# reinterpretcat/qwen3-rs

Hardware: NVIDIA B200
Metric: decode_tokens_per_s (higher is better)
Workload: dtype int8 weights x int8 activations, int32 group dots, f32 accumulate

## Files before the change

qwen3_rs_b200/csrc/q3_engine.cu:

```cuda
#include "../../include/qwen3_cuda.h"
#include "q3_kernels.cuh"
#include "q3_mega.cuh"
#include "q3_prefill.cuh"
#include "q3_sampler.cuh"
#include <cudaTypedefs.h>

#include <cuda_runtime.h>
#include <fcntl.h>
#include <math.h>
#include <stdarg.h>
#include <stdio.h>
#include <stdlib.h>
#include <string.h>
#include <sys/mman.h>
#include <sys/stat.h>
#include <unistd.h>

#include <string>
#include <vector>

using namespace q3;

static thread_local char g_err[1024] = "";
static int fail(int code, const char *fmt, ...) {
// ... 438 lines not shown
    }
    return 0;
}

template <class K>
static int allow_smem(K kernel, int bytes) {
    CK(cudaFuncSetAttribute(kernel, cudaFuncAttributeMaxDynamicSharedMemorySize, bytes));
    return 0;
}
static int prepare_exact_kernels() {
    int rc;
    if ((rc = allow_smem(k_rmsnorm_quant<32, true>, 65536))) return rc;
    if ((rc = allow_smem(k_rmsnorm_quant<64, true>, 65536))) return rc;
    if ((rc = allow_smem(k_rmsnorm_quant<128, true>, 65536))) return rc;
#define ALLOW_GEMV(GS)                                                      \
    if ((rc = allow_smem(k_gemv<GS, EPI_STORE, true, false>, 131072))) return rc;  \
    if ((rc = allow_smem(k_gemv<GS, EPI_QKV, true, false>, 131072))) return rc;    \
    if ((rc = allow_smem(k_gemv<GS, EPI_RESID, true, false>, 131072))) return rc;  \
    if ((rc = allow_smem(k_gemv<GS, EPI_SWIGLU, true, false>, 131072))) return rc; \
    if ((rc = allow_smem(k_gemv<GS, EPI_SWIGLU, true, true>, 131072))) return rc;  \
    if ((rc = allow_smem(k_gemv<GS, EPI_STORE, false, false>, 98304))) return rc;  \
    if ((rc = allow_smem(k_gemv<GS, EPI_QKV, false, false>, 98304))) return rc;    \
    if ((rc = allow_smem(k_gemv<GS, EPI_RESID, false, false>, 98304))) return rc;  \
    if ((rc = allow_smem(k_gemv<GS, EPI_SWIGLU, false, false>, 98304))) return rc; \
    if ((rc = allow_smem(k_gemv<GS, EPI_SWIGLU, false, true>, 98304))) return rc;
    ALLOW_GEMV(32)
    ALLOW_GEMV(64)
    ALLOW_GEMV(128)
#undef ALLOW_GEMV
    return 0;
}

static int pick_n_kt(int K, int gs) {
    for (int n = (K + MEGA_MAX_KT - 1) / MEGA_MAX_KT; n <= 64; n++)
        if (K % (n * gs) == 0 && (K / n) % 16 == 0 && K / n <= MEGA_MAX_KT) return n;
    return 0;
}

static int build_stream(q3_handle *h, MegaGemv &g, const std::vector<const DevQT *> &src, int units, int K, bool pair) {
    const int gs = h->cfg.group_size;
    g.units = units;
    g.K = K;
    g.n_kt = pick_n_kt(K, gs);
    if (!g.n_kt) return fail(Q3_EUNSUPPORTED, "no K tiling for K=%d gs=%d", K, gs);
    g.KT = K / g.n_kt;
    g.G = g.KT / gs;
    g.tile_bytes = g.KT + ((4 * g.G + 15) & ~15);
    const size_t rows = (size_t)units * (pair ? 2 : 1);
    g.layer_stride = (long long)(rows * g.n_kt * g.tile_bytes);
    uint8_t *buf = nullptr;
    int rc;
    if ((rc = dmalloc(h, (void **)&buf, (size_t)g.layer_stride * src.size()))) return rc;
    g.base = buf;
    for (size_t l = 0; l < src.size(); l++) {
        dim3 grid(units, g.n_kt);
        GS_DISPATCH(gs, (k_build_stream<GS><<<grid, 256, 0, h->stream>>>(src[l]->q, src[l]->s, buf + l * g.layer_stride, units, K,
                                                                        g.n_kt, h->num_sms, pair ? 1 : 0)));
    }
    CK(cudaGetLastError());
    return 0;
}

static PFN_cuTensorMapEncodeTiled_v12000 get_encode_fn();
static int make_map_kv(CUtensorMap *map, const float *base, size_t rows, int KV_l) {
    auto enc = get_encode_fn();
    if (!enc) return fail(Q3_ECUDA, "cuTensorMapEncodeTiled unavailable");
    cuuint64_t dims[2] = {(cuuint64_t)KV_l, (cuuint64_t)rows};
    cuuint64_t strides[1] = {(cuuint64_t)KV_l * 4};
    cuuint32_t box[2] = {(cuuint32_t)HEAD_DIM, (cuuint32_t)MEGA_KV_ROWS};
    cuuint32_t estr[2] = {1, 1};
    CUresult r = enc(map, CU_TENSOR_MAP_DATA_TYPE_FLOAT32, 2, const_cast<float *>(base), dims, strides, box, estr, CU_TENSOR_MAP_INTERLEAVE_NONE,
                     CU_TENSOR_MAP_SWIZZLE_NONE, CU_TENSOR_MAP_L2_PROMOTION_L2_128B, CU_TENSOR_MAP_FLOAT_OOB_FILL_NONE);
    if (r != CUDA_SUCCESS) return fail(Q3_ECUDA, "cuTensorMapEncodeTiled (KV cache) failed (%d) rows %zu KV %d", (int)r, rows, KV_l);
    return 0;
}

static int build_mega(q3_handle *h, const float *rms_att_all, const float *rms_ffn_all, const float *q_ln_all, const float *k_ln_all) {
    const q3_config &c = h->cfg;
    const int gs = c.group_size, L = c.n_layers, dim = c.dim;
    h->mega_ok = false;
    if (dim > MEGA_MAX_KT) { h->mega_why = "dim > 4096 (QKV/gate-up/lm_head phases need a single K tile)"; return 0; }
    if (!pick_n_kt(h->AH_l, gs) || !pick_n_kt(h->H_l, gs)) { h->mega_why = "no K tiling for o_proj/down"; return 0; }
    if (h->AH_l > 16384 || h->H_l > 16384 || dim > 16384) { h->mega_why = "activation vector > 16384"; return 0; }
    if (c.vocab_size % h->tp_size) { h->mega_why = "vocab not divisible by tp"; return 0; }
    if (h->layers[0].qkv.rows < h->num_sms || h->H_l < h->num_sms) { h->mega_why = "fewer qkv rows / FFN units than SMs"; return 0; }
    if (!get_encode_fn()) { h->mega_why = "cuTensorMapEncodeTiled unavailable"; return 0; }
    MegaArgs &a = h->margs;
    a = MegaArgs{};
    {
        int rck;
        if ((rck = make_map_kv(&a.map_k, h->kc, (size_t)L * c.seq_len, h->KV_l))) return rck;
        if ((rck = make_map_kv(&a.map_v, h->vc, (size_t)L * c.seq_len, h->KV_l))) return rck;
    }
    a.dim = dim; a.n_layers = L; a.n_heads_l = h->n_heads_l; a.n_kv_l = h->n_kv_l; a.AH_l = h->AH_l; a.KV_l = h->KV_l;
    a.H_l = h->H_l; a.seq_len = c.seq_len; a.tp_rank = h->tp_rank; a.tp_size = h->tp_size;
    a.vocab_l = c.vocab_size / h->tp_size;
    a.vocab_row0 = a.vocab_l * h->tp_rank;
    int rc;
    std::vector<const DevQT *> v;
    for (auto &W : h->layers) v.push_back(&W.qkv);
    if ((rc = build_stream(h, a.g[PH_QKV], v, h->layers[0].qkv.rows, dim, false))) return rc;
    v.clear();
    for (auto &W : h->layers) v.push_back(&W.wo);
    if ((rc = build_stream(h, a.g[PH_O], v, dim, h->AH_l, false))) return rc;
    v.clear();
    for (auto &W : h->layers) v.push_back(&W.w13);
    if ((rc = build_stream(h, a.g[PH_GU], v, h->H_l, dim, true))) return rc;
    v.clear();
    for (auto &W : h->layers) v.push_back(&W.w2);
    if ((rc = build_stream(h, a.g[PH_DN], v, dim, h->H_l, false))) return rc;
    DevQT head_slice = h->wcls;
    head_slice.q = h->wcls.q + (size_t)a.vocab_row0 * dim;
    head_slice.s = h->wcls.s + (size_t)a.vocab_row0 * (dim / gs);
    v.assign(1, &head_slice);
    if ((rc = build_stream(h, a.g[PH_HEAD], v, a.vocab_l, dim, false))) return rc;
    CK(cudaStreamSynchronize(h->stream));
    float *p;
    if ((rc = upload_f32(h, &p, rms_att_all, (size_t)L * dim))) return rc; a.rms_att = p;
    if ((rc = upload_f32(h, &p, rms_ffn_all, (size_t)L * dim))) return rc; a.rms_ffn = p;
    if ((rc = upload_f32(h, &p, q_ln_all, (size_t)L * HEAD_DIM))) return rc; a.q_ln = p;
    if ((rc = upload_f32(h, &p, k_ln_all, (size_t)L * HEAD_DIM))) return rc; a.k_ln = p;
    a.rms_final = h->rms_final;
    a.embed_q = h->embed.q; a.embed_s = h->embed.s; a.rope = h->rope; a.kc = h->kc; a.vc = h->vc;
    for (int i = 0; i < 2; i++) h->part_buf[i] = (unsigned long long *)(h->xchg + h->off_part[i]);
    {
        struct { unsigned long long **p; size_t words; } zones[] = {
            {&h->zq, (size_t)h->AH_l + 2 * (size_t)h->KV_l},
            {&h->za, (size_t)h->AH_l / 4 + (size_t)h->AH_l / gs},
            {&h->zh, (size_t)h->H_l},
            {&h->zr[0], (size_t)dim},
            {&h->zr[1], (size_t)dim}};
        for (auto &z : zones) {
            if ((rc = dmalloc(h, (void **)z.p, (z.words + 2) * 8))) return rc;
            CK(cudaMemset(*z.p, 0, (z.words + 2) * 8));
        }
    }
    h->d_best = (unsigned long long *)(h->xchg + h->off_best);
    h->d_flags = (unsigned int *)(h->xchg + h->off_flags);
    if ((rc = dmalloc(h, (void **)&h->d_bar, 64))) return rc;
    CK(cudaMemset(h->d_bar, 0, 64));
    if ((rc = dmalloc(h, (void **)&h->d_status, 64))) return rc;
    CK(cudaMemset(h->d_status, 0, 64));
    int *d_status = h->d_status;
    a.x = h->x;
    a.zq = h->zq; a.za = h->za; a.zh = h->zh; a.zr[0] = h->zr[0]; a.zr[1] = h->zr[1];
    a.attn_part = h->attn_part; a.att_cnt = h->att_cnt;
    a.bar = h->d_bar; a.status = d_status; a.tokpos = h->d_tokpos; a.history = h->d_history;
    for (int r = 0; r < MEGA_MAX_TP; r++) {
        a.part[0][r] = h->part_buf[0]; a.part[1][r] = h->part_buf[1];
        a.logits[r] = h->logits; a.best[r] = h->d_best; a.xbar[r] = (unsigned long long *)h->d_flags;
    }
    GS_DISPATCH(gs, KV_DISPATCH(h->kv_mul, (h->mega_fn = (void *)k_mega_decode<GS, KVM>)));
    if (!h->mega_fn) { h->mega_why = "no kernel for this GQA factor"; return 0; }
    const size_t slot = (size_t)MEGA_GW * (MEGA_MAX_KT + 4 * (MEGA_MAX_KT / gs));
    h->mega_smem = MEGA_NSTAGE * slot + MEGA_SCRATCH + 1024 + MEGA_MAX_KT * 4;
    CK(cudaFuncSetAttribute(h->mega_fn, cudaFuncAttributeMaxDynamicSharedMemorySize, (int)h->mega_smem));
    int occ = 0;
    CK(cudaOccupancyMaxActiveBlocksPerMultiprocessor(&occ, h->mega_fn, MEGA_THREADS, h->mega_smem));
    if (occ < 1) { h->mega_why = "megakernel does not fit on an SM"; return 0; }
    h->mega_ok = true;
    return 0;
}

static int launch_mega(q3_handle *h, int l0, int l1, bool from_embed, bool run_head, bool feedback, bool gather) {
    MegaArgs a = h->margs;
    a.layer0 = l0; a.layer1 = l1; a.from_embed = from_embed; a.run_head = run_head; a.feedback = feedback;
// ... 1399 lines not shown
```

qwen3_rs_b200/csrc/q3_mega.cuh:

```cuda
#pragma once
#include <cuda.h>

#include "q3_kernels.cuh"

namespace q3 {

#ifndef MEGA_GW_
#define MEGA_GW_ 8
#endif
constexpr int MEGA_GW = MEGA_GW_;
constexpr int MEGA_BATCH = 4 * MEGA_GW;
constexpr int MEGA_GROUPS = 2;
constexpr int MEGA_NCW = MEGA_GW * MEGA_GROUPS;
constexpr int MEGA_CTHREADS = MEGA_NCW * 32;
constexpr int MEGA_THREADS = MEGA_CTHREADS + 32 * MEGA_GROUPS;
#ifndef MEGA_NSTAGE_
#define MEGA_NSTAGE_ 4
#endif
constexpr int MEGA_NSTAGE = MEGA_NSTAGE_;
constexpr int MEGA_MAX_KT = 4096;
constexpr int MEGA_SCRATCH = 40960;
constexpr int MEGA_MAX_TP = 8;
constexpr int MEGA_MAX_SPLITS = ATTN_MAX_SPLITS;
constexpr int MEGA_EDGES = 6;

enum { PH_QKV = 0, PH_O = 1, PH_GU = 2, PH_DN = 3, PH_HEAD = 4 };

struct MegaGemv {
    const uint8_t *base;
    long long layer_stride;
    int units;
    int K, n_kt, KT, G;
    int tile_bytes;
};

constexpr int MEGA_KV_ROWS = 32;

struct MegaArgs {
    alignas(64) CUtensorMap map_k;
    alignas(64) CUtensorMap map_v;
    int dim, n_layers, n_heads_l, n_kv_l, AH_l, KV_l, H_l, vocab_l, vocab_row0, seq_len;
    int tp_rank, tp_size;
    MegaGemv g[5];
    const float *rms_att, *rms_ffn, *q_ln, *k_ln, *rms_final;
    const int8_t *embed_q;
    const float *embed_s;
    const float *rope;
    float *kc, *vc;
    float *x;
    unsigned long long *zq;
    unsigned long long *za;
    unsigned long long *zh;
    unsigned long long *zr[2];
    unsigned long long *part[2][MEGA_MAX_TP];
    float *attn_part;
    unsigned *att_cnt;
    float *logits[MEGA_MAX_TP];
    unsigned long long *best[MEGA_MAX_TP];
    unsigned long long *bar;
    unsigned long long bar_base;
    unsigned long long *xbar[MEGA_MAX_TP];
    unsigned long long xbar_base;
    int *tokpos, *history;
    int *status;
    int layer0, layer1, from_embed, run_head, feedback, gather_logits;
    unsigned ll_base;
    unsigned long long *prof;
};
constexpr int MEGA_PROF_EVENTS = 4096;
struct Prof {
    unsigned long long *row;
    int ev;
};
#define prof_mark(p, tag)                                                                                              \
    do {                                                                                                               \
        if (a.prof) {  \
            Prof &p_ = (p);                                                                                            \
            if (p_.row && p_.ev < MEGA_PROF_EVENTS - 1) p_.row[p_.ev++] = ((unsigned long long)clock64() << 8) | (unsigned)(tag); \
        }                                                                                                              \
    } while (0)

__device__ __forceinline__ uint32_t smem_u32(const void *p) { return (uint32_t)__cvta_generic_to_shared(p); }
__device__ __forceinline__ void mbar_init(uint64_t *bar, int count) {
    asm volatile("mbarrier.init.shared::cta.b64 [%0], %1;" ::"r"(smem_u32(bar)), "r"(count));
}
__device__ __forceinline__ void mbar_expect_tx(uint64_t *bar, uint32_t bytes) {
    asm volatile("mbarrier.arrive.expect_tx.shared::cta.b64 _, [%0], %1;" ::"r"(smem_u32(bar)), "r"(bytes) : "memory");
}
__device__ __forceinline__ void mbar_arrive(uint64_t *bar) {
    asm volatile("mbarrier.arrive.shared::cta.b64 _, [%0];" ::"r"(smem_u32(bar)) : "memory");
}
__device__ __forceinline__ bool mbar_try_wait(uint64_t *bar, uint32_t parity) {
    uint32_t ok;
    asm volatile("{\n.reg .pred p;\nmbarrier.try_wait.parity.shared::cta.b64 p, [%1], %2;\nselp.u32 %0, 1, 0, p;\n}"
                 : "=r"(ok)
                 : "r"(smem_u32(bar)), "r"(parity)
                 : "memory");
    return ok != 0;
}
__device__ __noinline__ void mbar_wait_slow(uint64_t *bar, uint32_t parity, int *status);
__device__ __forceinline__ void mbar_wait(uint64_t *bar, uint32_t parity, int *status) {
    if (mbar_try_wait(bar, parity)) return;
    mbar_wait_slow(bar, parity, status);
}
__device__ __noinline__ void mbar_wait_slow(uint64_t *bar, uint32_t parity, int *status) {
    long long t0 = clock64();
    unsigned spins = 0;
    while (!mbar_try_wait(bar, parity)) {
        if ((++spins & 4095u) == 0) {
            if (*(volatile int *)status) return;
            if (clock64() - t0 > 4000000000LL) {
                atomicExch(status, 2);
                return;
            }
        }
    }
}
__device__ __forceinline__ void bulk_g2s(void *dst, const void *src, uint32_t bytes, uint64_t *bar, uint64_t policy) {
    asm volatile(
        "cp.async.bulk.shared::cluster.global.mbarrier::complete_tx::bytes.L2::cache_hint [%0], [%1], %2, [%3], %4;" ::"r"(
            smem_u32(dst)),
        "l"(src), "r"(bytes), "r"(smem_u32(bar)), "l"(policy)
        : "memory");
}
__device__ __forceinline__ void tma_load_2d(void *dst, const CUtensorMap *map, int c0, int c1, uint64_t *bar) {
    asm volatile("cp.async.bulk.tensor.2d.shared::cluster.global.mbarrier::complete_tx::bytes [%0], [%1, {%2, %3}], [%4];" ::"r"(
                     smem_u32(dst)),
                 "l"(map), "r"(c0), "r"(c1), "r"(smem_u32(bar))
                 : "memory");
}
__device__ __forceinline__ void csync() { asm volatile("bar.sync 1, %0;" ::"n"(MEGA_CTHREADS) : "memory"); }
__device__ __forceinline__ float ldcg_f(const float *p) { return __ldcg(p); }
__device__ __forceinline__ float4 ldcg_f4(const float *p) { return __ldcg(reinterpret_cast<const float4 *>(p)); }

__device__ __forceinline__ unsigned ll_epoch(unsigned base, unsigned k) {
    unsigned long long s = (unsigned long long)base + k;
    if (s >= 0xFFFFFFFFull) s -= 0xFFFFFFFFull;
    return (unsigned)s + 1u;
}
__device__ __forceinline__ void ll_store_u32(unsigned long long *p, unsigned payload, unsigned epoch) {
    const unsigned long long w = ((unsigned long long)epoch << 32) | (unsigned long long)payload;
    asm volatile("st.relaxed.sys.global.b64 [%0], %1;" ::"l"(p), "l"(w) : "memory");
}
__device__ __forceinline__ void ll_store(unsigned long long *p, float v, unsigned epoch) { ll_store_u32(p, __float_as_uint(v), epoch); }
__device__ __forceinline__ void ll_load2(const unsigned long long *p, unsigned long long &x, unsigned long long &y) {
    asm volatile("ld.relaxed.sys.global.v2.b64 {%0,%1}, [%2];" : "=l"(x), "=l"(y) : "l"(p) : "memory");
}
__device__ __forceinline__ unsigned long long ll_load1(const unsigned long long *p) {
    unsigned long long x;
    asm volatile("ld.relaxed.sys.global.b64 %0, [%1];" : "=l"(x) : "l"(p) : "memory");
    return x;
}
__device__ __forceinline__ bool ll_ok(unsigned long long w, unsigned epoch) { return (unsigned)(w >> 32) == epoch; }
__device__ __noinline__ bool ll_give_up(const MegaArgs &a, unsigned &spins, int code) {
    if ((++spins & 255u) == 0) {
        if (*(volatile int *)a.status) return true;
        if (spins > (1u << 20)) {
            atomicExch(a.status, code);
            return true;
        }
    }
    return false;
}
__device__ __forceinline__ float4 ll_poll4(const MegaArgs &a, const unsigned long long *p, unsigned epoch, int code) {
    unsigned long long w0, w1, w2, w3;
    unsigned spins = 0;
    while (true) {
        ll_load2(p, w0, w1);
        ll_load2(p + 2, w2, w3);
        if (ll_ok(w0, epoch) && ll_ok(w1, epoch) && ll_ok(w2, epoch) && ll_ok(w3, epoch)) break;
        if (ll_give_up(a, spins, code)) break;
    }
    return make_float4(__uint_as_float((unsigned)w0), __uint_as_float((unsigned)w1), __uint_as_float((unsigned)w2), __uint_as_float((unsigned)w3));
}

__device__ __host__ __forceinline__ void cta_share(int units, int nctas, int c, int &start, int &count) {
    int base = units / nctas, rem = units % nctas;
    count = base + (c < rem ? 1 : 0);
    start = c * base + (c < rem ? c : rem);
}

template <int GS>
// ... 141 lines not shown
    for (int k = 0; k < MAXV; k++) {
        const int i4 = tid + k * MEGA_CTHREADS;
        v[k] = make_float4(0.f, 0.f, 0.f, 0.f);
        if (i4 < n4) {
            if (src == 0) {
                size_t base = (size_t)a.tokpos[0] * a.dim + (size_t)i4 * 4;
                char4 e = *reinterpret_cast<const char4 *>(a.embed_q + base);
                float sc = a.embed_s[base / GS];
                v[k] = make_float4((float)e.x * sc, (float)e.y * sc, (float)e.z * sc, (float)e.w * sc);
            } else if (src == 1) {
                v[k] = ldcg_f4(a.x + (size_t)i4 * 4);
            } else {
                v[k] = reinterpret_cast<const float4 *>(sx)[i4];
            }
        }
    }
    if (zone) {
        unsigned long long ww[MAXV][4];
        unsigned spins = 0;
        while (true) {
            bool ok = true;
#pragma unroll
            for (int k = 0; k < MAXV; k++) {
                const int i4 = tid + k * MEGA_CTHREADS;
                if (i4 < n4) {
                    ll_load2(zone + (size_t)i4 * 4, ww[k][0], ww[k][1]);
                    ll_load2(zone + (size_t)i4 * 4 + 2, ww[k][2], ww[k][3]);
                    ok = ok && ll_ok(ww[k][0], epoch) && ll_ok(ww[k][1], epoch) && ll_ok(ww[k][2], epoch) && ll_ok(ww[k][3], epoch);
                }
            }
            if (ok || ll_give_up(a, spins, 6)) break;
        }
#pragma unroll
        for (int k = 0; k < MAXV; k++) {
            if (tid + k * MEGA_CTHREADS < n4) {
                v[k].x = __fadd_rn(v[k].x, __uint_as_float((unsigned)ww[k][0]));
                v[k].y = __fadd_rn(v[k].y, __uint_as_float((unsigned)ww[k][1]));
                v[k].z = __fadd_rn(v[k].z, __uint_as_float((unsigned)ww[k][2]));
                v[k].w = __fadd_rn(v[k].w, __uint_as_float((unsigned)ww[k][3]));
            }
        }
    }
#pragma unroll
    for (int k = 0; k < MAXV; k++) {
        const int i4 = tid + k * MEGA_CTHREADS;
        if (i4 < n4) {
            reinterpret_cast<float4 *>(sx)[i4] = v[k];
            ss += __fmul_rn(v[k].x, v[k].x);
            ss += __fmul_rn(v[k].y, v[k].y);
            ss += __fmul_rn(v[k].z, v[k].z);
            ss += __fmul_rn(v[k].w, v[k].w);
        }
    }
    prof_mark(pr, 32);
    ss = warp_sum(ss);
    if (lane == 0) sred[warp] = ss;
    csync();
    float t = 0.0f;
#pragma unroll
    for (int i = 0; i < MEGA_NCW; i++) t += sred[i];
    const float f = __fdiv_rn(1.0f, sqrtf(__fadd_rn(__fdiv_rn(t, (float)a.dim), NORM_EPS)));
    prof_mark(pr, 33);
#pragma unroll
    for (int k = 0; k < MAXV; k++) {
        int i4 = tid + k * MEGA_CTHREADS;
        if (i4 - lane < n4) {
            float4 y = make_float4(0.f, 0.f, 0.f, 0.f);
            if (i4 < n4) {
                y.x = __fmul_rn(wv[k].x, __fmul_rn(f, v[k].x));
                y.y = __fmul_rn(wv[k].y, __fmul_rn(f, v[k].y));
                y.z = __fmul_rn(wv[k].z, __fmul_rn(f, v[k].z));
                y.w = __fmul_rn(wv[k].w, __fmul_rn(f, v[k].w));
            }
            uint32_t packed;
            float scale;
            quantize_group4<GS>(y, packed, scale);
            if (i4 < n4) {
                xq_store<GS>(sxq, i4, packed, KT, G);
                if ((i4 % (GS / 4)) == 0) sxs[i4 / (GS / 4)] = scale;
            }
        }
    }
    prof_mark(pr, 34);
    csync();
}

template <int GS>
__device__ __noinline__ void prologue_attn_poll(const MegaArgs &a, unsigned epoch, uint8_t *sxq, float *sxs) {
    const int tid = threadIdx.x;
    const int nq = a.AH_l >> 2, ng = a.AH_l / GS;
    unsigned spins = 0;
    for (int i = 2 * tid; i < nq; i += 2 * MEGA_CTHREADS) {
        unsigned long long x, y;
        while (true) {
            ll_load2(a.za + i, x, y);
            if ((ll_ok(x, epoch) && ll_ok(y, epoch)) || ll_give_up(a, spins, 7)) break;
        }
        *reinterpret_cast<uint2 *>(sxq + 4 * i) = make_uint2((unsigned)x, (unsigned)y);
    }
    for (int g = tid; g < ng; g += MEGA_CTHREADS) {
        unsigned long long x;
        while (true) {
            x = ll_load1(a.za + nq + g);
            if (ll_ok(x, epoch) || ll_give_up(a, spins, 7)) break;
        }
        sxs[g] = __uint_as_float((unsigned)x);
    }
    csync();
}

template <int GS>
__device__ __forceinline__ void quant_ll_one(const MegaArgs &a, const unsigned long long *z, unsigned epoch, int i4, int n4, unsigned long long (&w)[4],
                                             unsigned &spins, uint8_t *sxq, float *sxs, int KT, int G) {
    float4 y = make_float4(0.f, 0.f, 0.f, 0.f);
    if (i4 < n4) {
        while (!(ll_ok(w[0], epoch) && ll_ok(w[1], epoch) && ll_ok(w[2], epoch) && ll_ok(w[3], epoch))) {
            if (ll_give_up(a, spins, 8)) break;
            ll_load2(z + (size_t)i4 * 4, w[0], w[1]);
            ll_load2(z + (size_t)i4 * 4 + 2, w[2], w[3]);
        }
        y = make_float4(__uint_as_float((unsigned)w[0]), __uint_as_float((unsigned)w[1]), __uint_as_float((unsigned)w[2]), __uint_as_float((unsigned)w[3]));
    }
    uint32_t packed;
    float scale;
    quantize_group4<GS>(y, packed, scale);
    if (i4 < n4) {
        xq_store<GS>(sxq, i4, packed, KT, G);
        if ((i4 % (GS / 4)) == 0) sxs[i4 / (GS / 4)] = scale;
    }
}
template <int GS>
__device__ __noinline__ void prologue_quant_ll(const MegaArgs &a, const unsigned long long *z, unsigned epoch, int n, uint8_t *sxq, float *sxs, int KT, int G) {
    const int tid = threadIdx.x, lane = tid & 31;
    const int n4 = n >> 2;
    unsigned long long wa[4] = {0, 0, 0, 0}, wb[4] = {0, 0, 0, 0};
    unsigned spins = 0;
    int i4 = tid;
    if (i4 < n4) {
        ll_load2(z + (size_t)i4 * 4, wa[0], wa[1]);
        ll_load2(z + (size_t)i4 * 4 + 2, wa[2], wa[3]);
    }
#pragma unroll 1
    while (i4 - lane < n4) {
        int j4 = i4 + MEGA_CTHREADS;
        if (j4 < n4) {
            ll_load2(z + (size_t)j4 * 4, wb[0], wb[1]);
            ll_load2(z + (size_t)j4 * 4 + 2, wb[2], wb[3]);
        }
        quant_ll_one<GS>(a, z, epoch, i4, n4, wa, spins, sxq, sxs, KT, G);
        i4 = j4;
        if (!(i4 - lane < n4)) break;
        j4 = i4 + MEGA_CTHREADS;
        if (j4 < n4) {
            ll_load2(z + (size_t)j4 * 4, wa[0], wa[1]);
            ll_load2(z + (size_t)j4 * 4 + 2, wa[2], wa[3]);
        }
        quant_ll_one<GS>(a, z, epoch, i4, n4, wb, spins, sxq, sxs, KT, G);
        i4 = j4;
    }
    csync();
}

__device__ __forceinline__ float4 qk_norm_rope_pre(float4 v, float4 wv, float4 cs01, float4 cs23, int lane) {
    float ss = __fmul_rn(v.x, v.x);
    ss = __fadd_rn(ss, __fmul_rn(v.y, v.y));
    ss = __fadd_rn(ss, __fmul_rn(v.z, v.z));
    ss = __fadd_rn(ss, __fmul_rn(v.w, v.w));
    ss = warp_sum(ss);
    const float f = __fdiv_rn(1.0f, sqrtf(__fadd_rn(__fdiv_rn(ss, (float)HEAD_DIM), NORM_EPS)));
    float4 y;
    y.x = __fmul_rn(wv.x, __fmul_rn(f, v.x));
    y.y = __fmul_rn(wv.y, __fmul_rn(f, v.y));
    y.z = __fmul_rn(wv.z, __fmul_rn(f, v.z));
    y.w = __fmul_rn(wv.w, __fmul_rn(f, v.w));
    float4 o;
    o.x = __shfl_xor_sync(0xffffffffu, y.x, 16);
    o.y = __shfl_xor_sync(0xffffffffu, y.y, 16);
    o.z = __shfl_xor_sync(0xffffffffu, y.z, 16);
    o.w = __shfl_xor_sync(0xffffffffu, y.w, 16);
    float4 r;
    if (lane < 16) {
        r.x = __fsub_rn(__fmul_rn(y.x, cs01.x), __fmul_rn(o.x, cs01.y));
        r.y = __fsub_rn(__fmul_rn(y.y, cs01.z), __fmul_rn(o.y, cs01.w));
        r.z = __fsub_rn(__fmul_rn(y.z, cs23.x), __fmul_rn(o.z, cs23.y));
        r.w = __fsub_rn(__fmul_rn(y.w, cs23.z), __fmul_rn(o.w, cs23.w));
    } else {
        r.x = __fadd_rn(__fmul_rn(o.x, cs01.y), __fmul_rn(y.x, cs01.x));
        r.y = __fadd_rn(__fmul_rn(o.y, cs01.w), __fmul_rn(y.y, cs01.z));
        r.z = __fadd_rn(__fmul_rn(o.z, cs23.y), __fmul_rn(y.z, cs23.x));
        r.w = __fadd_rn(__fmul_rn(o.w, cs23.w), __fmul_rn(y.w, cs23.z));
// ... 271 lines not shown
#pragma unroll
            for (int j = 0; j < 4; j++) {
                const float c = __shfl_sync(0xffffffffu, cs, (s0 + j) & 31);
                As.x += pv[j].x * c;
                As.y += pv[j].y * c;
                As.z += pv[j].z * c;
                As.w += pv[j].w * c;
            }
        }
        publish_head<GS>(a, head, lane, As, Ls, ep_a);
    }
}

struct BarState {
    unsigned long long target;
    unsigned long long xtarget;
};

__device__ __noinline__ void grid_barrier(const MegaArgs &a, BarState &bs, bool cross, Prof &pr) {
    csync();
    prof_mark(pr, 40);
    const bool x = cross && a.tp_size > 1;
    if (threadIdx.x == 0) {
        long long t0 = clock64();
        volatile int *st = a.status;
        unsigned spins = 0;
        if (x) {
            __threadfence_system();
            for (int r = 0; r < a.tp_size; r++)
                asm volatile("red.relaxed.sys.global.add.u64 [%0], %1;" ::"l"(a.xbar[r]), "l"(1ULL) : "memory");
            while (true) {
                unsigned long long v;
                asm volatile("ld.acquire.sys.global.u64 %0, [%1];" : "=l"(v) : "l"(a.xbar[a.tp_rank]) : "memory");
                if (v >= bs.xtarget) break;
                if ((++spins & 1023u) == 0) {
                    if (*st) break;
                    if (clock64() - t0 > 8000000000LL) {
                        atomicExch(a.status, 3);
                        break;
                    }
                }
            }
        } else {
            asm volatile("red.release.gpu.global.add.u64 [%0], %1;" ::"l"(a.bar), "l"(1ULL) : "memory");
            while (true) {
                unsigned long long v;
                asm volatile("ld.acquire.gpu.global.u64 %0, [%1];" : "=l"(v) : "l"(a.bar) : "memory");
                if (v >= bs.target) break;
                if ((++spins & 1023u) == 0) {
                    if (*st) break;
                    if (clock64() - t0 > 4000000000LL) {
                        atomicExch(a.status, 1);
                        break;
                    }
                }
            }
        }
    }
    if (x) bs.xtarget += (unsigned long long)a.tp_size * gridDim.x;
    else bs.target += gridDim.x;
    prof_mark(pr, 41);
    csync();
}

struct PhaseGeom {
    const uint8_t *seg;
    int start, count;
};
struct MegaShared {
    int start[5], count[5];
    long long seg_off[5], seg_len[5];
    unsigned long long *part[2][MEGA_MAX_TP];
    float *logits[MEGA_MAX_TP];
    unsigned long long *best[MEGA_MAX_TP];
};
__device__ __forceinline__ PhaseGeom phase_geom(const MegaArgs &a, const MegaShared &sh, int ph, int layer) {
    PhaseGeom pg;
    pg.start = sh.start[ph];
    pg.count = sh.count[ph];
    pg.seg = a.g[ph].base + (long long)layer * a.g[ph].layer_stride + sh.seg_off[ph];
    return pg;
}

template <int GS, int KVMUL>
__global__ void __launch_bounds__(MEGA_THREADS, 1) k_mega_decode(const __grid_constant__ MegaArgs a) {
    extern __shared__ __align__(1024) uint8_t mega_smem[];
    uint8_t *smem = mega_smem;
    const int slot_bytes = MEGA_GW * (MEGA_MAX_KT + 4 * (MEGA_MAX_KT / GS));
    uint8_t *ring = smem;
    uint8_t *scratch = smem + MEGA_NSTAGE * slot_bytes;
    uint8_t *sxq = scratch;
    float *sxs = reinterpret_cast<float *>(scratch + 16384);
    float *sred = reinterpret_cast<float *>(scratch + 16384 + 2048);
    uint64_t *full = reinterpret_cast<uint64_t *>(scratch + MEGA_SCRATCH);
    uint64_t *empty = full + MEGA_GROUPS * MEGA_NSTAGE;
    MegaShared &sh = *reinterpret_cast<MegaShared *>(scratch + MEGA_SCRATCH + 192);
    static_assert(192 + sizeof(MegaShared) <= 1024, "MegaShared outgrew its slot");
    float *sx = reinterpret_cast<float *>(scratch + MEGA_SCRATCH + 1024);
    volatile unsigned *issued = reinterpret_cast<volatile unsigned *>(scratch + MEGA_SCRATCH + 128);
    const int tid = threadIdx.x, lane = tid & 31, warp = tid >> 5;

    if (tid == 0) {
        for (int s = 0; s < MEGA_NSTAGE; s++) {
            mbar_init(&full[s], 1);
            mbar_init(&full[MEGA_NSTAGE + s], 1);
            mbar_init(&empty[s], MEGA_GW);
            issued[s] = 0;
        }
        asm volatile("fence.mbarrier_init.release.cluster;" ::: "memory");
#pragma unroll 1
        for (int ph = 0; ph < 5; ph++) {
            int st, cn;
            cta_share(a.g[ph].units, gridDim.x, blockIdx.x, st, cn);
            const long long per_unit = (long long)(ph == PH_GU ? 2 : 1) * a.g[ph].n_kt * a.g[ph].tile_bytes;
            sh.start[ph] = st;
            sh.count[ph] = cn;
            sh.seg_off[ph] = st * per_unit;
            sh.seg_len[ph] = cn * per_unit;
        }
    }
    if (tid < MEGA_MAX_TP) {
        sh.part[0][tid] = a.part[0][tid];
        sh.part[1][tid] = a.part[1][tid];
        sh.logits[tid] = a.logits[tid];
        sh.best[tid] = a.best[tid];
    }
    __syncthreads();

    const int L0 = a.layer0, L1 = a.layer1;

    if (warp >= MEGA_NCW) {
        if (lane != 0) return;
        const int pw = warp - MEGA_NCW;
        uint64_t policy;
        asm volatile("createpolicy.fractional.L2::evict_first.b64 %0, 1.0;" : "=l"(policy));
        unsigned it = 0;
        Prof pr;
        pr.row = (a.prof && pw == 0) ? a.prof + (size_t)(gridDim.x + blockIdx.x) * MEGA_PROF_EVENTS : nullptr;
        pr.ev = 0;
        auto push = [&](const uint8_t *src, int nr, int tile_bytes, int owner) {
            if (owner != pw) {
                it++;
                return;
            }
            const int slot = it % MEGA_NSTAGE;
            const uint32_t bytes = (uint32_t)nr * tile_bytes;
            {
                const unsigned use = it / MEGA_NSTAGE;
                long long t0 = clock64();
                while (issued[slot] != use) {
                    if (clock64() - t0 > 4000000000LL) { atomicExch(a.status, 4); break; }
                }
            }
            mbar_wait(&empty[slot], ((it / MEGA_NSTAGE) & 1) ^ 1, a.status);
            uint64_t *fb = &full[owner * MEGA_NSTAGE + slot];
            mbar_expect_tx(fb, bytes);
            bulk_g2s(ring + (size_t)slot * slot_bytes, src, bytes, fb, policy);
            __threadfence_block();
            issued[slot] = it / MEGA_NSTAGE + 1;
            prof_mark(pr, 64 + slot);
            it++;
        };
        const int ppos = a.tokpos[1];
        const int pns = mega_nsplit(ppos, a.n_kv_l, gridDim.x);
        const bool has_item = (int)blockIdx.x < a.n_kv_l * pns;
        const int pkvh = blockIdx.x % a.n_kv_l, psplit = blockIdx.x / a.n_kv_l;
        const int pper = (ppos + 1 + pns - 1) / pns;
        const int pt0 = psplit * pper, pt1 = pt0 + pper < ppos + 1 ? pt0 + pper : ppos + 1;
        auto kvpush = [&](int layer) {
            if (!has_item) return;
            for (int t = pt0, si = 0; t < pt1; t += MEGA_KV_ROWS, si++) {
                const int owner = si & 1;
                if (owner != pw) {
                    it++;
                    continue;
                }
                const int slot = it % MEGA_NSTAGE;
                {
                    const unsigned use = it / MEGA_NSTAGE;
                    long long tw = clock64();
                    while (issued[slot] != use) {
                        if (clock64() - tw > 4000000000LL) { atomicExch(a.status, 4); break; }
                    }
                }
                mbar_wait(&empty[slot], ((it / MEGA_NSTAGE) & 1) ^ 1, a.status);
                uint64_t *fb = &full[owner * MEGA_NSTAGE + slot];
                uint8_t *dst = ring + (size_t)slot * slot_bytes;
                mbar_expect_tx(fb, 2 * MEGA_KV_ROWS * HEAD_DIM * 4);
                tma_load_2d(dst, &a.map_k, pkvh * HEAD_DIM, layer * a.seq_len + t, fb);
                tma_load_2d(dst + MEGA_KV_ROWS * HEAD_DIM * 4, &a.map_v, pkvh * HEAD_DIM, layer * a.seq_len + t, fb);
                __threadfence_block();
// ... 2 lines not shown
                it++;
            }
        };
        auto plain = [&](int ph, int layer) {
            const MegaGemv &g = a.g[ph];
            PhaseGeom pg = phase_geom(a, sh, ph, layer);
            const uint8_t *src = pg.seg;
            for (int b0 = 0; b0 < pg.count; b0 += MEGA_BATCH) {
                int nb = pg.count - b0 < MEGA_BATCH ? pg.count - b0 : MEGA_BATCH;
                for (int kt = 0; kt < g.n_kt; kt++)
                    for (int s = 0, si = 0; s < nb; s += MEGA_GW, si++) {
                        int nr = nb - s < MEGA_GW ? nb - s : MEGA_GW;
                        push(src, nr, g.tile_bytes, si & 1);
                        src += (size_t)nr * g.tile_bytes;
                    }
            }
        };
        auto pairs = [&](int layer) {
            const MegaGemv &g = a.g[PH_GU];
            PhaseGeom pg = phase_geom(a, sh, PH_GU, layer);
            const uint8_t *src = pg.seg;
            for (int p0 = 0, bi = 0; p0 < pg.count; p0 += MEGA_GW, bi++) {
                int np = pg.count - p0 < MEGA_GW ? pg.count - p0 : MEGA_GW;
                for (int half = 0; half < 2; half++) {
                    push(src, np, g.tile_bytes, bi & 1);
                    src += (size_t)np * g.tile_bytes;
                }
            }
        };
        for (int l = L0; l < L1; l++) {
            plain(PH_QKV, l);
            kvpush(l);
            plain(PH_O, l);
            pairs(l);
            plain(PH_DN, l);
        }
        if (a.run_head) plain(PH_HEAD, 0);
        if (pr.row) pr.row[MEGA_PROF_EVENTS - 1] = (unsigned long long)pr.ev;
        return;
    }

    unsigned it = 0;
    BarState bs;
    bs.target = a.bar_base + gridDim.x;
    bs.xtarget = a.xbar_base + (unsigned long long)a.tp_size * gridDim.x;
    const int pos = a.tokpos[1];
    const int grp = warp / MEGA_GW, wl = warp % MEGA_GW;
    Prof pr;
    pr.row = (a.prof && (tid == 0 || tid == MEGA_GW * 32)) ? a.prof + (size_t)((tid ? 2 * gridDim.x : 0) + blockIdx.x) * MEGA_PROF_EVENTS : nullptr;
    pr.ev = 0;
    unsigned fullp = 0;
    uint64_t *myfull = full + grp * MEGA_NSTAGE;
    XRegs<GS> xr;
    prof_mark(pr, 0);
    long long best = (long long)0x8000000000000000LL;
    const int n_layer_steps = 5 * (L1 - L0);
    const int n_steps = n_layer_steps + (a.run_head ? 1 : 0);
    const int nsplit = mega_nsplit(pos, a.n_kv_l, gridDim.x);

    for (int step = 0; step < n_steps; step++) {
        const bool head = step >= n_layer_steps;
        const int l = head ? 0 : L0 + step / 5;
        const int kind = head ? 5 : step % 5;
        const unsigned ep_step = ll_epoch(a.ll_base, head ? (unsigned)(MEGA_EDGES * (L1 - L0)) : (unsigned)(MEGA_EDGES * (l - L0) + kind));
        const unsigned ep_prev = ll_epoch(a.ll_base, (unsigned)(MEGA_EDGES * (l - L0) + kind - 1));
        int ph = PH_QKV;
        if (kind == 0 || kind == 3 || kind == 5) {
            const float *w = kind == 0 ? a.rms_att + (size_t)l * a.dim : kind == 3 ? a.rms_ffn + (size_t)l * a.dim : a.rms_final;
            const bool emb = kind == 0 && l == L0 && a.from_embed;
            const bool pending = kind == 3 || (kind == 0 ? l > L0 : L1 > L0);
            ph = kind == 0 ? PH_QKV : kind == 3 ? PH_GU : PH_HEAD;
            const unsigned ep_rows = kind == 3 ? ep_prev : ll_epoch(a.ll_base, (unsigned)(MEGA_EDGES * ((kind == 0 ? l - 1 : L1 - 1) - L0) + 4));
            prologue_norm<GS>(a, w, emb ? 0 : (pending ? 2 : 1), pending ? a.zr[kind == 3 ? 0 : 1] : nullptr, ep_rows, sxq, sxs, sred, sx,
                              a.g[ph].KT, a.g[ph].G, pr);
        } else if (kind == 1) {
            if ((int)blockIdx.x < a.n_kv_l * nsplit) {
                RingPos rp{it, fullp};
                attention_item<GS, KVMUL>(a, l, pos, blockIdx.x % a.n_kv_l, blockIdx.x / a.n_kv_l, nsplit, scratch, ep_prev, ep_step, pr, rp,
                                          smem_u32(ring), slot_bytes, myfull, empty);
                it = rp.it;
                fullp = rp.fullp;
            }
        } else if (kind == 2) {
            prologue_attn_poll<GS>(a, ep_prev, sxq, sxs);
            ph = PH_O;
        } else {
            prologue_quant_ll<GS>(a, a.zh, ep_prev, a.H_l, sxq, sxs, a.g[PH_DN].KT, a.g[PH_DN].G);
            ph = PH_DN;
        }
        prof_mark(pr, 1 + 3 * kind);
        if (kind != 1) {
            const MegaGemv &g = a.g[ph];
            const int start = sh.start[ph], count = sh.count[ph];
            const bool full_blocks = (g.G & 31) == 0;
            const uint32_t ring_s = smem_u32(ring);
            if (kind == 3) {
                const unsigned ep_h = ep_step;
                load_x<GS>(xr, sxq, sxs, 0, g.KT, g.G, lane);
                for (int p0 = 0, bi = 0; p0 < count; p0 += MEGA_GW, bi++) {
                    const int np = count - p0 < MEGA_GW ? count - p0 : MEGA_GW;
                    if ((bi & 1) != grp) {
                        it += 2;
                        continue;
                    }
                    float gate = 0.0f, up = 0.0f;
                    for (int half = 0; half < 2; half++) {
                        const int slot = it % MEGA_NSTAGE;
                        mbar_wait(&myfull[slot], (fullp >> slot) & 1, a.status);
                        fullp ^= 1u << slot;
                        prof_mark(pr, 48 + slot);
                        {
                            const uint32_t tile = ring_s + slot * slot_bytes + wl * g.tile_bytes;
                            float v = full_blocks ? tile_dot<GS, true>(tile, xr, g.KT, g.G, lane) : tile_dot<GS, false>(tile, xr, g.KT, g.G, lane);
                            gate = half == 0 ? v : gate;
                            up = half == 0 ? up : v;
                        }
                        __syncwarp();
                        if (lane == 0) mbar_arrive(&empty[slot]);
                        it++;
                    }
                    if (wl < np && lane == 0) {
                        float sw = __fmul_rn(gate, __fdiv_rn(1.0f, __fadd_rn(1.0f, expf(-gate))));
                        ll_store(a.zh + start + p0 + wl, __fmul_rn(sw, up), ep_h);
                    }
                }
            } else {
                const unsigned ep_out = ep_step;
                for (int b0 = 0; b0 < count; b0 += MEGA_BATCH) {
                    const int nb = count - b0 < MEGA_BATCH ? count - b0 : MEGA_BATCH;
                    float acc0 = 0.f, acc1 = 0.f;
                    for (int kt = 0; kt < g.n_kt; kt++) {
                        load_x<GS>(xr, sxq, sxs, kt, g.KT, g.G, lane);
                        prof_mark(pr, 58);
                        for (int sidx = 0; MEGA_GW * sidx < nb; sidx++) {
                            if ((sidx & 1) == grp) {
                                const int slot = it % MEGA_NSTAGE;
                                mbar_wait(&myfull[slot], (fullp >> slot) & 1, a.status);
                                fullp ^= 1u << slot;
                                prof_mark(pr, 48 + slot);
                                {
                                    const uint32_t tile = ring_s + slot * slot_bytes + wl * g.tile_bytes;
                                    float v = full_blocks ? tile_dot<GS, true>(tile, xr, g.KT, g.G, lane) : tile_dot<GS, false>(tile, xr, g.KT, g.G, lane);
                                    v = (MEGA_GW * sidx + wl < nb) ? v : 0.0f;
                                    acc0 += sidx < 2 ? v : 0.0f;
                                    acc1 += sidx < 2 ? 0.0f : v;
                                    prof_mark(pr, 59);
                                }
                                __syncwarp();
                                if (lane == 0) mbar_arrive(&empty[slot]);
                            }
                            it++;
                        }
                    }
                    if (lane == 0) {
                        for (int j = 0; j < 2; j++) {
                            const int sidx = grp + 2 * j;
                            if (MEGA_GW * sidx + wl >= nb) break;
                            const int r = start + b0 + MEGA_GW * sidx + wl;
                            const float v = j == 0 ? acc0 : acc1;
                            if (kind == 0) {
                                ll_store(a.zq + r, v, ep_out);
                            } else if (kind == 2 || kind == 4) {
                                if (a.tp_size == 1) {
                                    ll_store(a.zr[kind == 2 ? 0 : 1] + r, v, ep_out);
                                } else {
                                    unsigned long long *const *dst = sh.part[kind == 2 ? 0 : 1];
#pragma unroll 1
                                    for (int p = 0; p < a.tp_size; p++) ll_store(dst[p] + (size_t)a.tp_rank * a.dim + r, v, ep_out);
                                }
                            } else {
                                const int row = a.vocab_row0 + r;
                                sh.logits[a.tp_rank][row] = v;
                                if (a.gather_logits) {
#pragma unroll 1
                                    for (int p = 0; p < a.tp_size; p++)
                                        if (p != a.tp_rank && ((a.gather_logits >> p) & 1)) sh.logits[p][row] = v;
                                }
                                long long key = ((long long)total_key(v) << 32) | (unsigned)row;
                                best = key > best ? key : best;
                            }
                        }
                    }
                }
                if ((kind == 2 || kind == 4) && a.tp_size > 1) {
                    const unsigned long long *src = sh.part[kind == 2 ? 0 : 1][a.tp_rank];
                    for (int idx = tid; idx < count; idx += MEGA_CTHREADS) {
                        const int r = start + idx;
                        unsigned long long w[MEGA_MAX_TP];
                        unsigned spins = 0;
                        while (true) {
                            bool ok = true;
#pragma unroll
                            for (int p = 0; p < MEGA_MAX_TP; p++) {
                                if (p < a.tp_size) {
                                    w[p] = ll_load1(src + (size_t)p * a.dim + r);
                                    ok = ok && ll_ok(w[p], ep_out);
                                }
                            }
                            if (ok || ll_give_up(a, spins, 10)) break;
                        }
                        float s = __uint_as_float((unsigned)w[0]);
#pragma unroll
                        for (int p = 1; p < MEGA_MAX_TP; p++)
                            if (p < a.tp_size) s = __fadd_rn(s, __uint_as_float((unsigned)w[p]));
                        ll_store(a.zr[kind == 2 ? 0 : 1] + r, s, ep_out);
                    }
                }
            }
        }
        prof_mark(pr, 2 + 3 * kind);
        if (kind == 5) {
            long long *sbest = reinterpret_cast<long long *>(sred + 32);
            if (lane == 0) sbest[warp] = best;
            csync();
            if (tid == 0) {
                for (int w = 1; w < MEGA_NCW; w++) best = sbest[w] > best ? sbest[w] : best;
#pragma unroll 1
                for (int p = 0; p < a.tp_size; p++) sh.best[p][(size_t)a.tp_rank * gridDim.x + blockIdx.x] = (unsigned long long)best;
            }
        }
        if (kind == 2 || kind == 4) {
            const float *wn = kind == 2 ? a.rms_ffn + (size_t)l * a.dim : (l + 1 < L1 ? a.rms_att + (size_t)(l + 1) * a.dim : a.rms_final);
            if (tid * 32 < a.dim) asm volatile("prefetch.global.L2 [%0];" ::"l"(wn + tid * 32));
        } else if (kind == 0 && tid < 12) {
            const float *wn = tid < 4 ? a.q_ln + (size_t)l * HEAD_DIM + tid * 32 : tid < 8 ? a.k_ln + (size_t)l * HEAD_DIM + (tid - 4) * 32
                                                                                   : a.rope + (size_t)pos * HEAD_DIM + (tid - 8) * 32;
            asm volatile("prefetch.global.L2 [%0];" ::"l"(wn));
        }
        if (kind == 5) grid_barrier(a, bs, true, pr);
        else csync();
        prof_mark(pr, 3 + 3 * kind);
    }

    if (pr.row) pr.row[MEGA_PROF_EVENTS - 1] = (unsigned long long)pr.ev;
    if (a.run_head) {
        if (blockIdx.x == 0 && warp == 0) {
            long long b = (long long)0x8000000000000000LL;
            const int n = a.tp_size * gridDim.x;
            for (int i = lane; i < n; i += 32) {
                long long k = (long long)__ldcg(sh.best[a.tp_rank] + i);
                b = k > b ? k : b;
            }
#pragma unroll
            for (int o = 16; o > 0; o >>= 1) {
                long long other = __shfl_xor_sync(0xffffffffu, b, o);
                b = other > b ? other : b;
            }
            if (lane == 0) {
                int tok = (int)(b & 0xffffffffLL);
                a.tokpos[2] = tok;
                if (a.feedback) {
                    a.tokpos[0] = tok;
                    a.tokpos[1] = pos + 1;
                    a.history[a.tokpos[3]] = tok;
                    a.tokpos[3] += 1;
                }
            }
        }
    } else if (blockIdx.x == 0 && L1 > L0) {
        const unsigned ep = ll_epoch(a.ll_base, (unsigned)(MEGA_EDGES * (L1 - 1 - L0) + 4));
        for (int i4 = tid; i4 < (a.dim >> 2); i4 += MEGA_CTHREADS) {
            float4 v = reinterpret_cast<const float4 *>(sx)[i4];
            const float4 d = ll_poll4(a, a.zr[1] + (size_t)i4 * 4, ep, 6);
            v.x = __fadd_rn(v.x, d.x);
            v.y = __fadd_rn(v.y, d.y);
            v.z = __fadd_rn(v.z, d.z);
            v.w = __fadd_rn(v.w, d.w);
            reinterpret_cast<float4 *>(a.x)[i4] = v;
        }
    }
}

}
```

Before: 457.6.

## Overlap o_proj GEMV with per-head attention output arrival via mbarriers

Replaces the blocking attention-output poll before o_proj with a fused step. Each head's quantized activations are written to shared memory as they arrive, and a per-head mbarrier is signalled. Consumer warps then compute the partial dot products for each K block as soon as its head is ready, instead of waiting for the whole vector. This adds a new eligibility check that disables the mega kernel when o_proj needs more than one K tile or more than ring-size rows per SM, and it introduces more complex spin-wait logic.

Result: slower. 435.3 (median of 6 runs) (-4.9%).

```diff
diff --git a/qwen3_rs_b200/csrc/q3_engine.cu b/qwen3_rs_b200/csrc/q3_engine.cu
--- a/qwen3_rs_b200/csrc/q3_engine.cu
+++ b/qwen3_rs_b200/csrc/q3_engine.cu
@@ -544,6 +544,10 @@
     if (dim > MEGA_MAX_KT) { h->mega_why = "dim > 4096 (QKV/gate-up/lm_head phases need a single K tile)"; return 0; }
     if (!pick_n_kt(h->AH_l, gs) || !pick_n_kt(h->H_l, gs)) { h->mega_why = "no K tiling for o_proj/down"; return 0; }
     if (h->AH_l > 16384 || h->H_l > 16384 || dim > 16384) { h->mega_why = "activation vector > 16384"; return 0; }
+    if (pick_n_kt(h->AH_l, gs) != 1 || (dim + h->num_sms - 1) / h->num_sms > MEGA_NSTAGE * MEGA_GW) {
+        h->mega_why = "o_proj share of a CTA does not fit the ring at once (needs n_heads * 128 <= 4096 and <= 32 rows per SM)";
+        return 0;
+    }
     if (c.vocab_size % h->tp_size) { h->mega_why = "vocab not divisible by tp"; return 0; }
     if (h->layers[0].qkv.rows < h->num_sms || h->H_l < h->num_sms) { h->mega_why = "fewer qkv rows / FFN units than SMs"; return 0; }
     if (!get_encode_fn()) { h->mega_why = "cuTensorMapEncodeTiled unavailable"; return 0; }
diff --git a/qwen3_rs_b200/csrc/q3_mega.cuh b/qwen3_rs_b200/csrc/q3_mega.cuh
--- a/qwen3_rs_b200/csrc/q3_mega.cuh
+++ b/qwen3_rs_b200/csrc/q3_mega.cuh
@@ -98,6 +98,14 @@
                  : "memory");
     return ok != 0;
 }
+__device__ __forceinline__ bool mbar_test_wait(uint64_t *bar, uint32_t parity) {
+    uint32_t ok;
+    asm volatile("{\n.reg .pred p;\nmbarrier.test_wait.parity.shared::cta.b64 p, [%1], %2;\nselp.u32 %0, 1, 0, p;\n}"
+                 : "=r"(ok)
+                 : "r"(smem_u32(bar)), "r"(parity)
+                 : "memory");
+    return ok != 0;
+}
 __device__ __noinline__ void mbar_wait_slow(uint64_t *bar, uint32_t parity, int *status);
 __device__ __forceinline__ void mbar_wait(uint64_t *bar, uint32_t parity, int *status) {
     if (mbar_try_wait(bar, parity)) return;
@@ -405,30 +413,6 @@
         }
     }
     prof_mark(pr, 34);
-    csync();
-}
-
-template <int GS>
-__device__ __noinline__ void prologue_attn_poll(const MegaArgs &a, unsigned epoch, uint8_t *sxq, float *sxs) {
-    const int tid = threadIdx.x;
-    const int nq = a.AH_l >> 2, ng = a.AH_l / GS;
-    unsigned spins = 0;
-    for (int i = 2 * tid; i < nq; i += 2 * MEGA_CTHREADS) {
-        unsigned long long x, y;
-        while (true) {
-            ll_load2(a.za + i, x, y);
-            if ((ll_ok(x, epoch) && ll_ok(y, epoch)) || ll_give_up(a, spins, 7)) break;
-        }
-        *reinterpret_cast<uint2 *>(sxq + 4 * i) = make_uint2((unsigned)x, (unsigned)y);
-    }
-    for (int g = tid; g < ng; g += MEGA_CTHREADS) {
-        unsigned long long x;
-        while (true) {
-            x = ll_load1(a.za + nq + g);
-            if (ll_ok(x, epoch) || ll_give_up(a, spins, 7)) break;
-        }
-        sxs[g] = __uint_as_float((unsigned)x);
-    }
     csync();
 }
 
@@ -866,6 +850,124 @@
     return pg;
 }
 
+__device__ __forceinline__ void store_row_parallel(const MegaArgs &a, const MegaShared &sh, int which, int r, float v, unsigned epoch) {
+    if (a.tp_size == 1) {
+        ll_store(a.zr[which] + r, v, epoch);
+    } else {
+        unsigned long long *const *dst = sh.part[which];
+#pragma unroll 1
+        for (int p = 0; p < a.tp_size; p++) ll_store(dst[p] + (size_t)a.tp_rank * a.dim + r, v, epoch);
+    }
+}
+
+template <int GS>
+__device__ __forceinline__ void oproj_step(const MegaArgs &a, const MegaShared &sh, unsigned epoch, unsigned ep_out, uint8_t *sxq, float *sxs,
+                                           uint64_t *hbar, unsigned hpar, uint32_t ring_s, int slot_bytes, uint64_t *myfull, uint64_t *empty,
+                                           unsigned &it, unsigned &fullp) {
+    constexpr int CPG = XRegs<GS>::CPG, NBLK = XRegs<GS>::NBLK, HG = HEAD_DIM / GS;
+    const int tid = threadIdx.x, lane = tid & 31, warp = tid >> 5, grp = warp / MEGA_GW, wl = warp % MEGA_GW;
+    const MegaGemv &g = a.g[PH_O];
+    const int nb = sh.count[PH_O], nq = a.AH_l >> 2;
+    uint32_t tile[2];
+    bool row[2];
+#pragma unroll
+    for (int j = 0; j < 2; j++) {
+        const int sidx = grp + 2 * j, slot = (it + sidx) % MEGA_NSTAGE;
+        tile[j] = ring_s + slot * slot_bytes + wl * g.tile_bytes;
+        row[j] = MEGA_GW * sidx + wl < nb;
+        if (MEGA_GW * sidx < nb) {
+            mbar_wait(&myfull[slot], (fullp >> slot) & 1, a.status);
+            fullp ^= 1u << slot;
+        }
+    }
+    unsigned todo = (2 * tid < nq ? 1u : 0u) | (tid < g.G ? 2u : 0u);
+    int qhead = 0;
+    {
+        const int byte = 8 * tid, b = byte / (32 * GS);
+        const int ngb = g.G - 32 * b > 32 ? 32 : g.G - 32 * b;
+        if (todo & 1) qhead = (32 * b + ((byte - b * 32 * GS) >> 4) % ngb) / HG;
+    }
+    unsigned need = 0;
+#pragma unroll
+    for (int b = 0; b < NBLK; b++)
+        if (32 * b + lane < g.G) need |= 1u << b;
+    float t0[NBLK], t1[NBLK];
+#pragma unroll
+    for (int b = 0; b < NBLK; b++) t0[b] = t1[b] = 0.0f;
+    unsigned long long w0 = 0, w1 = 0, ws = 0;
+    const long long tstart = clock64();
+    unsigned spins = 0;
+    while (todo | need) {
+        if (todo & 1) ll_load2(a.za + 2 * tid, w0, w1);
+        if (todo & 2) ws = ll_load1(a.za + nq + tid);
+#pragma unroll
+        for (int b = 0; b < NBLK; b++) {
+            if (((need >> b) & 1) && mbar_test_wait(&hbar[(32 * b + lane) / HG], hpar)) {
+                need &= ~(1u << b);
+                const int ngb = g.G - 32 * b > 32 ? 32 : g.G - 32 * b;
+                const uint32_t xa = smem_u32(sxq) + b * 32 * GS + lane * 16;
+                int4 x[CPG];
+#pragma unroll
+                for (int p = 0; p < CPG; p++) x[p] = lds128(xa + p * ngb * 16);
+                const float xs = sxs[32 * b + lane];
+#pragma unroll
+                for (int j = 0; j < 2; j++) {
+                    if (!row[j]) continue;
+                    const uint32_t wa = tile[j] + b * 32 * GS + lane * 16;
+                    int4 w[CPG];
+#pragma unroll
+                    for (int p = 0; p < CPG; p++) w[p] = lds128(wa + p * ngb * 16);
+                    const float wsc = lds_f32(tile[j] + g.KT + (32 * b + lane) * 4);
+                    int d0 = 0, d1 = 0;
+#pragma unroll
+                    for (int p = 0; p < CPG; p += 2) {
+                        d0 = dot16(w[p], x[p], d0);
+                        d1 = dot16(w[p + 1], x[p + 1], d1);
+                    }
+                    const float t = __fmul_rn(__fmul_rn((float)(d0 + d1), wsc), xs);
+                    if (j == 0) t0[b] = t;
+                    else t1[b] = t;
+                }
+            }
+        }
+        if ((todo & 1) && ll_ok(w0, epoch) && ll_ok(w1, epoch)) {
+            *reinterpret_cast<uint2 *>(sxq + 8 * tid) = make_uint2((unsigned)w0, (unsigned)w1);
+            mbar_arrive(&hbar[qhead]);
+            todo &= ~1u;
+        }
+        if ((todo & 2) && ll_ok(ws, epoch)) {
+            sxs[tid] = __uint_as_float((unsigned)ws);
+            mbar_arrive(&hbar[tid / HG]);
+            todo &= ~2u;
+        }
+        if ((todo | need) && (++spins & 255u) == 0) {
+            if (*(volatile int *)a.status) break;
+            if (clock64() - tstart > 4000000000LL) {
+                atomicExch(a.status, 7);
+                break;
+            }
+        }
+    }
+    __syncwarp();
+    float acc0 = 0.0f, acc1 = 0.0f;
+#pragma unroll
+    for (int b = 0; b < NBLK; b++) {
+        acc0 = __fadd_rn(acc0, t0[b]);
+        acc1 = __fadd_rn(acc1, t1[b]);
+    }
+    const float v0 = warp_sum(acc0), v1 = warp_sum(acc1);
+    __syncwarp();
+    if (lane == 0) {
+#pragma unroll
+        for (int j = 0; j < 2; j++) {
+            const int sidx = grp + 2 * j;
+            if (MEGA_GW * sidx < nb) mbar_arrive(&empty[(it + sidx) % MEGA_NSTAGE]);
+            if (row[j]) store_row_parallel(a, sh, 0, sh.start[PH_O] + MEGA_GW * sidx + wl, j == 0 ? v0 : v1, ep_out);
+        }
+    }
+    it += (nb + MEGA_GW - 1) / MEGA_GW;
+}
+
 template <int GS, int KVMUL>
 __global__ void __launch_bounds__(MEGA_THREADS, 1) k_mega_decode(const __grid_constant__ MegaArgs a) {
     extern __shared__ __align__(1024) uint8_t mega_smem[];
@@ -879,7 +981,8 @@
     uint64_t *full = reinterpret_cast<uint64_t *>(scratch + MEGA_SCRATCH);
     uint64_t *empty = full + MEGA_GROUPS * MEGA_NSTAGE;
     MegaShared &sh = *reinterpret_cast<MegaShared *>(scratch + MEGA_SCRATCH + 192);
-    static_assert(192 + sizeof(MegaShared) <= 1024, "MegaShared outgrew its slot");
+    static_assert(192 + sizeof(MegaShared) <= 768, "MegaShared outgrew its slot");
+    uint64_t *hbar = reinterpret_cast<uint64_t *>(scratch + MEGA_SCRATCH + 768);
     float *sx = reinterpret_cast<float *>(scratch + MEGA_SCRATCH + 1024);
     volatile unsigned *issued = reinterpret_cast<volatile unsigned *>(scratch + MEGA_SCRATCH + 128);
     const int tid = threadIdx.x, lane = tid & 31, warp = tid >> 5;
@@ -891,6 +994,7 @@
             mbar_init(&empty[s], MEGA_GW);
             issued[s] = 0;
         }
+        for (int h = 0; h < a.n_heads_l; h++) mbar_init(&hbar[h], 16 + HEAD_DIM / GS);
         asm volatile("fence.mbarrier_init.release.cluster;" ::: "memory");
 #pragma unroll 1
         for (int ph = 0; ph < 5; ph++) {
@@ -1059,14 +1163,14 @@
                 fullp = rp.fullp;
             }
         } else if (kind == 2) {
-            prologue_attn_poll<GS>(a, ep_prev, sxq, sxs);
+            oproj_step<GS>(a, sh, ep_prev, ep_step, sxq, sxs, hbar, (unsigned)(l - L0) & 1u, smem_u32(ring), slot_bytes, myfull, empty, it, fullp);
             ph = PH_O;
         } else {
             prologue_quant_ll<GS>(a, a.zh, ep_prev, a.H_l, sxq, sxs, a.g[PH_DN].KT, a.g[PH_DN].G);
             ph = PH_DN;
         }
         prof_mark(pr, 1 + 3 * kind);
-        if (kind != 1) {
+        if (kind != 1 && kind != 2) {
             const MegaGemv &g = a.g[ph];
             const int start = sh.start[ph], count = sh.count[ph];
             const bool full_blocks = (g.G & 31) == 0;
@@ -1137,14 +1241,8 @@
                             const float v = j == 0 ? acc0 : acc1;
                             if (kind == 0) {
                                 ll_store(a.zq + r, v, ep_out);
-                            } else if (kind == 2 || kind == 4) {
-                                if (a.tp_size == 1) {
-                                    ll_store(a.zr[kind == 2 ? 0 : 1] + r, v, ep_out);
-                                } else {
-                                    unsigned long long *const *dst = sh.part[kind == 2 ? 0 : 1];
-#pragma unroll 1
-                                    for (int p = 0; p < a.tp_size; p++) ll_store(dst[p] + (size_t)a.tp_rank * a.dim + r, v, ep_out);
-                                }
+                            } else if (kind == 4) {
+                                store_row_parallel(a, sh, 1, r, v, ep_out);
                             } else {
                                 const int row = a.vocab_row0 + r;
                                 sh.logits[a.tp_rank][row] = v;
@@ -1159,30 +1257,30 @@
                         }
                     }
                 }
-                if ((kind == 2 || kind == 4) && a.tp_size > 1) {
-                    const unsigned long long *src = sh.part[kind == 2 ? 0 : 1][a.tp_rank];
-                    for (int idx = tid; idx < count; idx += MEGA_CTHREADS) {
-                        const int r = start + idx;
-                        unsigned long long w[MEGA_MAX_TP];
-                        unsigned spins = 0;
-                        while (true) {
-                            bool ok = true;
-#pragma unroll
-                            for (int p = 0; p < MEGA_MAX_TP; p++) {
-                                if (p < a.tp_size) {
-                                    w[p] = ll_load1(src + (size_t)p * a.dim + r);
-                                    ok = ok && ll_ok(w[p], ep_out);
-                                }
-                            }
-                            if (ok || ll_give_up(a, spins, 10)) break;
+            }
+        }
+        if ((kind == 2 || kind == 4) && a.tp_size > 1) {
+            const unsigned long long *src = sh.part[kind == 2 ? 0 : 1][a.tp_rank];
+            for (int idx = tid; idx < sh.count[ph]; idx += MEGA_CTHREADS) {
+                const int r = sh.start[ph] + idx;
+                unsigned long long w[MEGA_MAX_TP];
+                unsigned spins = 0;
+                while (true) {
+                    bool ok = true;
+#pragma unroll
+                    for (int p = 0; p < MEGA_MAX_TP; p++) {
+                        if (p < a.tp_size) {
+                            w[p] = ll_load1(src + (size_t)p * a.dim + r);
+                            ok = ok && ll_ok(w[p], ep_step);
                         }
-                        float s = __uint_as_float((unsigned)w[0]);
-#pragma unroll
-                        for (int p = 1; p < MEGA_MAX_TP; p++)
-                            if (p < a.tp_size) s = __fadd_rn(s, __uint_as_float((unsigned)w[p]));
-                        ll_store(a.zr[kind == 2 ? 0 : 1] + r, s, ep_out);
                     }
-                }
+                    if (ok || ll_give_up(a, spins, 10)) break;
+                }
+                float s = __uint_as_float((unsigned)w[0]);
+#pragma unroll
+                for (int p = 1; p < MEGA_MAX_TP; p++)
+                    if (p < a.tp_size) s = __fadd_rn(s, __uint_as_float((unsigned)w[p]));
+                ll_store(a.zr[kind == 2 ? 0 : 1] + r, s, ep_step);
             }
         }
         prof_mark(pr, 2 + 3 * kind);
```
